# Chanuk-Yang/Deep_Continuous_Fusion_for_Multi-Sensor_3D_Object_Detection

Hardware: AMD Instinct MI355X
Metric: frames/sec (train step) 100k-pt LiDAR + 1242x375 RGB (higher is better)
Workload: dtype bf16; 1 GPU; cfg2: grid 32x704x800, 100000 pts/frame, 1242x375 RGB, ResNet-18 image stream, K=3 fusion x4 sites, eval-mode BN (reference F4), batch 2/GPU; global_batch=2, parallelism=dp1, loss_sampling=compat, conv_chain=False

## Files before the change

### deep_continuous_fusion_for_multi-sensor_3d_object_detection_amd/_hip.py

```python
import ctypes
import os
import subprocess

import numpy as np
import torch

_HERE = os.path.dirname(os.path.abspath(__file__))
LIB_PATH = os.environ.get("DCF_HIP_LIB") or os.path.join(_HERE, "libdcf_hip.so")
CSRC = os.path.join(_HERE, "csrc")

F32, BF16, F16 = 0, 1, 2
VOXEL_COMPAT, VOXEL_ACCUM, VOXEL_COMPAT_ROUNDS, VOXEL_OCCUPANCY = 0, 1, 2, 3
PROJ_COMPAT, PROJ_CORRECT = 0, 1

c_int, c_float, c_i64, c_size_t, c_void_p = ctypes.c_int, ctypes.c_float, ctypes.c_int64, ctypes.c_size_t, ctypes.c_void_p
P = c_void_p

SIGNATURES = {
    "dcf_last_error": (ctypes.c_char_p, []),
    "dcf_version": (c_int, []),
    "dcf_set_option": (c_int, [ctypes.c_char_p, ctypes.c_char_p]),
    "dcf_prof_enable": (c_int, [c_int]),
    "dcf_prof_reset": (c_int, []),
    "dcf_prof_calibrate": (c_int, [P, c_int]),
    "dcf_prof_read": (c_int, [P, P, P, P, c_int]),
    "dcf_prof_read2": (c_int, [P, P, P, P, P, c_int]),
    "dcf_compact_workspace_bytes": (c_size_t, [c_int]),
    "dcf_range_filter": (c_int, [P, c_int, P, P, P, P, P, P]),
    "dcf_voxelize_workspace_bytes": (c_size_t, [c_int, c_int, c_int]),
    "dcf_voxelize": (c_int, [P, c_int, P, P, c_int, c_int, c_int, c_int, P, P, P]),
    "dcf_voxelize_batch": (c_int, [P, P, c_int, P, P, c_int, c_int, c_int, P, P, P]),
    "dcf_voxelize_batch_nhwc": (c_int, [c_int, P, P, c_int, P, P, c_int, c_int, c_int, P, P, P]),
    "dcf_project_filter": (c_int, [P, c_int, P, P, c_float, c_float, c_int, P, P, P, P, P, P]),
    "dcf_project_filter_batch": (c_int, [P, P, c_int, P, P, c_float, c_float, c_int, P, P, c_int, P, P, P]),
    "dcf_knn_workspace_bytes": (c_size_t, [c_int, c_int, c_int]),
    "dcf_knn_bev": (c_int, [P, P, c_int, c_int, c_int, c_int, c_int, c_float, c_float, c_float, c_float, c_float, P, P, P]),
    "dcf_knn_bev_batch": (c_int, [P, P, c_int, c_int, c_int, c_int, c_int, c_int, c_float, c_float, c_float, c_float, c_float, P, P, c_size_t, P]),
    "dcf_knn_bev_sites": (c_int, [P, P, c_int, c_int, c_int, P, c_int, c_float, c_float, c_float, c_float, c_float, P]),
    "dcf_knn_bev_batch_shared": (c_int, [P, P, c_int, c_int, c_int, c_int, c_int, c_int, c_int, c_int, c_int, c_float, c_float, c_float, c_float, c_float, P, P, c_size_t, P, c_size_t, P]),
    "dcf_nchw_to_nhwc": (c_int, [c_int, P, P, c_int, c_int, c_int, c_int, P]),
    "dcf_nhwc_to_nchw": (c_int, [c_int, P, P, c_int, c_int, c_int, c_int, P]),
    "dcf_image_to_nhwc4": (c_int, [c_int, P, P, c_int, c_int, c_int, P]),
    "dcf_conv2d_fwd": (c_int, [c_int, P, P, P, P, P] + [c_int] * 12 + [P]),
    "dcf_conv2d_fwd_rowscale": (c_int, [c_int, P, P, P, P, P, P] + [c_int] * 12 + [P]),
    "dcf_conv2d_dgrad": (c_int, [c_int, P, P, P, P, P] + [c_int] * 11 + [P]),
    "dcf_conv2d_dgrad_halfres": (c_int, [c_int, P, P, P, P, P, P] + [c_int] * 11 + [P]),
    "dcf_conv3x3_chain_supported": (c_int, [c_int] * 6),
    "dcf_conv3x3_chain_workspace_bytes": (c_size_t, [c_int] * 6),
    "dcf_conv3x3_chain": (c_int, [c_int, P, c_int, c_int, c_int, c_int, c_int, c_int, P, P]),
    "dcf_fp8_act_scale": (c_int, [c_float, P]),
    "dcf_cast_fp8": (c_int, [c_int, P, P, P, P, c_i64, P]),
    "dcf_weight_prep_fp8": (c_int, [P, P, c_int, c_int, P, P, P, P, P, c_float, P]),
    "dcf_conv2d_fwd_fp8": (c_int, [c_int, P, P, P, P, P, P, P, P, P, P] + [c_int] * 12 + [P]),
    "dcf_conv2d_wgrad_splits": (c_int, [c_int] * 8),
    "dcf_conv2d_wgrad": (c_int, [c_int, P, P, P, P, c_int] + [c_int] * 11 + [P]),
    "dcf_conv2d_wgrad_groupable": (c_int, [c_int] * 10),
    "dcf_conv2d_wgrad_group": (c_int, [P, c_int, P]),
    "dcf_stem7x7_fwd": (c_int, [c_int, P, P, P, P] + [c_int] * 7 + [P]),
    "dcf_stem7x7_wgrad": (c_int, [c_int, P, P, P, P, c_int] + [c_int] * 6 + [P]),
    "dcf_weight_prep": (c_int, [c_int, P, c_int, P, P, P, P, c_float, P]),
    "dcf_wgrad_finalize": (c_int, [P, c_int, c_int, P, P, P, P, P, P, c_float, P]),
    "dcf_eval_score_filter": (c_int, [P, c_int, c_int, c_int, c_float, c_int, P, P, P]),
    "dcf_eval_nms_workspace_bytes": (c_size_t, [c_int]),
    "dcf_eval_nms": (c_int, [P, P, c_int, c_int, ctypes.c_double, P, P, P, P]),
    "dcf_eval_match": (c_int, [P, c_int, P, c_int, P, c_int, P, P]),
    "dcf_wgrad_finalize_rows": (c_int, [P, c_int, P, P, P, P, P, P, P, c_float, P]),
    "dcf_bn_workspace_bytes": (c_size_t, [c_int]),
    "dcf_bn_train_fwd": (c_int, [c_int, P, P, P, P, P, P, P, P, P, c_i64, c_int, c_float, c_float, c_int, P, P]),
    "dcf_bn_train_bwd": (c_int, [c_int, P, P, P, P, P, P, P, P, c_i64, c_int, P, P]),
    "dcf_relu_bwd_chansum": (c_int, [c_int, P, P, P, c_i64, c_int, c_int, P]),
    "dcf_resize_bilinear_fwd": (c_int, [c_int, P, P, P] + [c_int] * 7 + [P]),
    "dcf_resize_bilinear_bwd": (c_int, [c_int, P, P] + [c_int] * 7 + [P]),
    "dcf_maxpool3x3s2_fwd": (c_int, [c_int, P, P] + [c_int] * 6 + [P]),
    "dcf_maxpool3x3s2_bwd": (c_int, [c_int, P, P, P, P] + [c_int] * 6 + [P]),
    "dcf_maxpool3x3s2_fwd_idx": (c_int, [c_int, P, P, P] + [c_int] * 6 + [P]),
    "dcf_maxpool3x3s2_bwd_idx": (c_int, [c_int, P, P, P] + [c_int] * 6 + [P]),
    "dcf_head_fwd": (c_int, [c_int, P, c_int, P, P, c_int, c_int, c_int, P]),
    "dcf_head_bwd": (c_int, [c_int, P, c_int, P, P, P, P, c_int, c_int, c_int, P]),
    "dcf_point_sample_fwd": (c_int, [c_int, P, c_int, c_int, c_int, P, P, c_int, P, P]),
    "dcf_point_sample_bwd": (c_int, [c_int, P, c_int, c_int, c_int, P, P, c_int, P, P]),
    "dcf_point_sample_fwd_batch": (c_int, [c_int, P, c_int, c_int, c_int, P, c_i64, P, c_int, P, c_int, P]),
    "dcf_point_sample_bwd_batch": (c_int, [c_int, P, c_int, c_int, c_int, P, c_i64, P, c_int, P, c_int, P]),
    "dcf_fusion_gather_fwd_batch": (c_int, [c_int, P, c_i64, P, c_i64, P, c_int, c_int, c_int, c_int, c_float, c_float, c_float, c_float, P, P, c_int, P, P, c_int, P]),
    "dcf_fusion_gather_bwd_inv_batch": (c_int, [c_int, P, c_i64, P, c_i64, P, P, c_i64, P, P, c_int, c_int, c_int, c_int, c_float, c_float, c_float, c_float, P, P, c_int, P, P, P, P, P, c_int, P]),
    "dcf_fusion_gather_fwd": (c_int, [c_int, P, P, P, c_int, c_int, c_int, c_int, c_float, c_float, c_float, c_float, P, P, c_int, P, P, P]),
    "dcf_fusion_gather_bwd": (c_int, [c_int, P, P, P, c_int, c_int, c_int, c_int, c_float, c_float, c_float, c_float, P, P, c_int, P, P, P, P, P]),
    "dcf_fusion_invert_workspace_bytes": (c_size_t, [c_int, c_int]),
    "dcf_fusion_invert": (c_int, [P, c_int, c_int, c_int, P, P, P, P, P]),
    "dcf_fusion_gather_bwd_pts": (c_int, [c_int, P, P, P, c_int, P, P, c_int, c_int, c_int, c_int, c_float, c_float, c_float, c_float, P, P, c_int, P, P, P, P, P]),
    "dcf_fusion_gather_bwd_workspace_bytes": (c_size_t, [c_int]),
    "dcf_fusion_gather_bwd_direct_workspace_bytes": (c_size_t, [c_int, c_int, c_int]),
    "dcf_fusion_gather_bwd_direct_batch": (c_int, [c_int, P, c_i64, P, c_i64, P, P, c_i64, P, P, c_int, c_int, c_int, c_int, c_float, c_float, c_float, c_float, P, P, c_int, P, P, P, P, P, P, c_int, P]),
    "dcf_fusion_gather_bwd_inv": (c_int, [c_int, P, P, P, P, P, P, c_int, c_int, c_int, c_int, c_float, c_float, c_float, c_float, P, P, c_int, P, P, P, P, P, P]),
    "dcf_rowscale_bias_fwd": (c_int, [c_int, P, P, P, c_i64, c_int, P]),
    "dcf_rowscale_bias_bwd": (c_int, [c_int, P, P, P, c_i64, c_int, P]),
    "dcf_relu_mask_rowscale_bwd": (c_int, [c_int, P, P, P, P, P, c_i64, c_int, P]),
    "dcf_cast": (c_int, [c_int, P, c_int, P, c_i64, P]),
    "dcf_loss_fwd_bwd": (c_int, [P, c_i64, P, c_i64, P, P, P, c_int, c_int, c_float, c_int, P, P, c_i64, P, c_i64, P]),
    "dcf_loss_sample_rand": (ctypes.c_uint32, [ctypes.c_uint64, c_int, c_int, c_int, c_int]),
# ... 187 lines not shown
```

### deep_continuous_fusion_for_multi-sensor_3d_object_detection_amd/backend_hip.py

```python
import ctypes
import os

import numpy as np
import torch

from . import _hip as H
from . import ops

BN_EPS = 1e-5


class HipBackend(object):
    def __init__(self, plan, params, grads, buffers, dtype, fp8_min_cin=0, fp8_min_blocks=512):
        if not params.is_cuda:
            raise H.DcfError("the HIP hot path needs CUDA/HIP tensors (got %s); there is no CPU fallback" % params.device)
        H.lib()
        self.plan, self.params, self.grads, self.buffers = plan, params, grads, buffers
        self.dtype = H.dtype_code(dtype)
        self.tdtype = H.torch_dtype(self.dtype)
        self.es = 4 if self.dtype == H.F32 else 2
        self.dev = params.device
        self._fus_dws = {}
        self._wtab = {}
        self._chain_ok, self._chain_ws, self._chain_tab = {}, {}, {}
# ... 327 lines not shown
    def can_chain(self, shape, n):
        if not self.chain_enabled or n < 2 or self.bn_train or self.has_fp8 or self.dtype == H.F32:
            return False
        if os.environ.get("DCF_CHAIN") != "force":
            import torch.distributed as dist
            if dist.is_available() and dist.is_initialized() and dist.get_world_size() > 1:
                return False
        key = tuple(shape)
        ok = self._chain_ok.get(key)
        if ok is None:
            B, Hh, W, C = key
            ok = self._chain_ok[key] = ops.conv3x3_chain_supported(self.dtype, B, Hh, W, C, 1)
        return ok

    def _chain(self, x, layers, flip):
        B, Hh, W, C = x.shape
        key = (B, Hh, W, C)
        ws = self._chain_ws.get(key)
        if ws is None:
            ws = self._chain_ws[key] = ops.conv3x3_chain_workspace(self.dtype, B, Hh, W, C, H.CHAIN_MAX_LAYERS, x.device)
        outs, cur, pos = [], x, 0
        while pos < len(layers):
            part = layers[pos:pos + H.CHAIN_MAX_LAYERS]
            fix = []
            for (w, sh, r, m, relu) in part:
                r = (outs[r] if r < pos else r - pos) if type(r) is int else r
                m = (outs[m] if m < pos else m - pos) if type(m) is int else m
                fix.append((w, sh, r, m, relu))
            tab = self._chain_tab.get(len(fix))
            if tab is None:
                tab = self._chain_tab[len(fix)] = (H.ChainLayer * len(fix))()
            got = ops.conv3x3_chain(self.dtype, cur, fix, flip, ws, tab)
            outs.extend(got)
            cur = got[-1]
            pos += len(part)
        return outs

    def chain_fwd(self, x, specs):
        outs = self._chain(x, [(self._wbase + L.wfwd_off, self._shift(L), r, None, relu) for (L, r, relu) in specs], 0)
        shp = (x.shape[0], x.shape[1], x.shape[2])
        for (L, _, _) in specs:
            L.out_shape = shp
        return outs

    def chain_dgrad(self, g, specs):
        for (L, _, _) in specs:
            if L.wdgrad_off < 0:
                raise H.DcfError("layer %s was planned without an input gradient" % L.name)
        return self._chain(g, [(self._wbase + L.wdgrad_off, None, r, m, False) for (L, r, m) in specs], 1)

    def shortcut_dgrad(self, Ld, dd, L1, g1, in_shape, mask=None):
        if L1.wdgrad_off < 0 or Ld.wdgrad_off < 0:
            raise H.DcfError("layer %s was planned without an input gradient" % L1.name)
        B, Hq, Wq, _ = dd.shape
        gq = ops.conv2d_dgrad(self.dtype, dd, self._w(Ld, True), None, (B, Hq, Wq, in_shape[3]), 1, 1, 1, 0)
        return ops.conv2d_dgrad_halfres(self.dtype, g1, self._w(L1, True), None, gq, in_shape, L1.kh, L1.kw, L1.stride, L1.pad, mask)

    def _gs(self, L):
        return self._gsbase + 4 * L.gsum_off if (L.bn is not None and not self.bn_train) else None

    def _flush_wgrads(self):
        q = self._wq
        if not q:
            return
        key = tuple([t[0].idx for t in q])
        ent = self._wtab.get(key)
        shapes = [t[1].shape for t in q]
        sig = (self.bn_train, self._slbase, self._gsbase, tuple([(t[0].nsplit, t[0].slab_off, t[0].gsum_off) for t in q]))
        if ent is None or ent[1] != shapes or ent[2] != sig:
            items = (H.WgradItem * len(q))()
            for i, (L, x, gy) in enumerate(q):
                B, Hh, W, Cin = x.shape
                items[i] = H.WgradItem(self.dtype, L.nsplit, 0, 0, self._slbase + 4 * L.slab_off, self._gs(L), B, Hh, W, Cin, L.cout_pad, L.kh, L.kw, L.stride, L.pad, 0)
            if len(self._wtab) > 16:
                self._wtab.clear()
            ent = self._wtab[key] = (items, shapes, sig)
        items = ent[0]
        for i, (L, x, gy) in enumerate(q):
            it = items[i]
            it.x = x.data_ptr()
            it.gy = gy.data_ptr()
        H.call("dcf_conv2d_wgrad_group", ctypes.addressof(items), len(q), H.stream_ptr())
        self._wq = []

    _wq = []
    _fus_ws = None
    _gp_pool = None
    _group = os.environ.get("DCF_WGRAD_GROUP", "1") != "0"
    _fusion_pts = os.environ.get("DCF_FUSION_PTS", "0") == "1"
    _fusion_direct = os.environ.get("DCF_FUSION_DIRECT", "1") != "0"

    deterministic = False
    _det_ws = None

    def _det_workspace(self, key, make):
        if self._det_ws is None:
            self._det_ws = {}
        ws = self._det_ws.get(key)
        if ws is None:
            ws = self._det_ws[key] = make()
        return ws

    def conv_wgrad(self, L, x, gy, defer=True):
        if self._group and defer and L.kind != "stem":
            q = self.__dict__.get("_wq")
            if q is None:
                q = self._wq = []
            q.append((L, x, gy))
            return
# ... 181 lines not shown
```

### deep_continuous_fusion_for_multi-sensor_3d_object_detection_amd/engine.py

```python
import os

import numpy as np
import torch

FUSION_INV = os.environ.get("DCF_FUSION_INV", "1")
FUSED_SITE_MASK = os.environ.get("DCF_FUSED_SITE_MASK", "1") != "0"
HALFRES_SHORTCUT = os.environ.get("DCF_HALFRES_SHORTCUT", "1") != "0"


class ConvLayer(object):

    def __init__(self, idx, name, cin, cout, kh, kw, stride, pad, bn=None, kind="conv", need_dgrad=True, names=None):
        self.idx, self.name, self.bn, self.kind = idx, name, bn, kind
        self.cin, self.cout, self.kh, self.kw, self.stride, self.pad = cin, cout, kh, kw, stride, pad
        self.cout_pad = (cout + 31) // 32 * 32
        self.need_dgrad = need_dgrad
        self.names = names or [name]
        self.w_off = self.gamma_off = self.beta_off = self.mean_off = self.var_off = -1
        self.out_shape = None

    @property
    def taps(self):
        return self.kh * self.kw

# ... 23 lines not shown
    @staticmethod
    def physical_shape(shape, layout):
        if layout == "ohwi":
            O, I, kh, kw = shape
            return (O, kh, kw, I)
        if layout == "stem":
            return (shape[0], 7, 8, 4)
        return tuple(shape)

    @staticmethod
    def view(flat, shape, off, n, layout):
        seg = flat[off:off + n]
        if layout == "ohwi":
            O, I, kh, kw = shape
            return seg.view(O, kh, kw, I).permute(0, 3, 1, 2)
        if layout == "stem":
            return seg.view(shape[0], 7, 8, 4)[:, :, :7, :3].permute(0, 3, 1, 2)
        return seg.view(shape)


class Block(object):

    def __init__(self, conv1, conv2, down=None):
        self.conv1, self.conv2, self.down = conv1, conv2, down
        self.saved = None
        self.next_conv = None

    def forward(self, K, x, save=True):
        r = K.conv_fwd(self.down, x, None, False) if self.down is not None else x
        y1 = K.conv_fwd(self.conv1, x, None, True, self.conv2)
        y = K.conv_fwd(self.conv2, y1, r, True, self.next_conv)
        x._f8 = y1._f8 = None
        self.saved = (x, y1, y) if save else None
        return y

    def backward(self, K, g, extra=None, need_gx=True, g_masked=False, prev=None):
        x, y1, y = self.saved
        self.saved = None
        g2 = g if g_masked else K.relu_mask(g, y)
        d2 = K.bn_bwd(self.conv2, g2)
        K.conv_wgrad(self.conv2, y1, d2)
        g1 = K.bn_bwd(self.conv1, K.conv_dgrad(self.conv2, d2, tuple(y1.shape), None, y1))
        return self.backward_tail(K, x, g2, g1, extra, need_gx, prev)

    def backward_tail(self, K, x, g2, g1, extra, need_gx, prev):
        K.conv_wgrad(self.conv1, x, g1)
        pm = x if prev is not None else None
        if self.down is not None:
            dd = K.bn_bwd(self.down, g2)
            K.conv_wgrad(self.down, x, dd)
            if not need_gx:
                return None
            d, c = self.down, self.conv1
            if (extra is None and HALFRES_SHORTCUT and d.kh == 1 and d.kw == 1 and d.stride == 2 and d.pad == 0
                    and c.kh == 3 and c.stride == 2 and c.pad == 1):
                return K.shortcut_dgrad(d, dd, c, g1, tuple(x.shape), pm)
            gx = K.conv_dgrad(self.down, dd, tuple(x.shape), extra)
            return K.conv_dgrad(self.conv1, g1, tuple(x.shape), gx, pm)
        if not need_gx:
            return None
        assert extra is None, "an identity-shortcut block cannot take an extra gradient"
        return K.conv_dgrad(self.conv1, g1, tuple(x.shape), g2, pm)


def blocks_forward(K, blocks, x, save=True):
    n = len(blocks)
    ok = (n >= 1 and getattr(K, "can_chain", None) is not None and all(type(b) is Block for b in blocks)
          and all(b.down is None and b.conv1.stride == 1 for b in blocks[1:]))
    if ok:
        b0 = blocks[0]
        strided = b0.down is not None or b0.conv1.stride != 1 or b0.conv1.cin != b0.conv1.cout
        nchain = 2 * n - 1 if strided else 2 * n
        B, Hh, W, _ = x.shape
        s0 = b0.conv1.stride
        shape = (B, (Hh + 2 - 3) // s0 + 1, (W + 2 - 3) // s0 + 1, b0.conv1.cout) if strided else tuple(x.shape)
        ok = nchain >= 2 and all(L.kh == 3 and L.kw == 3 and L.pad == 1 and L.cout == L.cout_pad == shape[3]
                                 for b in blocks for L in (b.conv1, b.conv2)) and K.can_chain(shape, nchain)
    if not ok:
        for b in blocks:
            x = b.forward(K, x, save)
        return x
    specs, ins = [], []
    if strided:
        r = K.conv_fwd(b0.down, x, None, False) if b0.down is not None else x
        y1 = K.conv_fwd(b0.conv1, x, None, True)
        x0 = y1
        specs.append((b0.conv2, r, True))
        first = 1
    else:
        x0 = x
        first = 0
    xin = len(specs) - 1
    for b in blocks[first:]:
        specs.append((b.conv1, None, True))
        specs.append((b.conv2, xin if xin >= 0 else x, True))
        xin = len(specs) - 1
    outs = K.chain_fwd(x0, specs)
    if save:
        k = 0
        if strided:
            b0.saved = (x, y1, outs[0])
            k = 1
        prev = outs[0] if strided else x
        for b in blocks[first:]:
            b.saved = (prev, outs[k], outs[k + 1])
            prev = outs[k + 1]
            k += 2
    else:
        for b in blocks:
# ... 488 lines not shown
```

### deep_continuous_fusion_for_multi-sensor_3d_object_detection_amd/ops.py

```python
import ctypes

import numpy as np
import torch

from . import _hip as H


def _chk(t, name):
    if not (isinstance(t, torch.Tensor) and t.is_cuda and t.is_contiguous()):
        raise H.DcfError("%s must be a contiguous CUDA tensor" % name)
    return t


def conv_out_size(n, k, s, p):
    return (n + 2 * p - k) // s + 1


def nchw_to_nhwc(x, dtype):
    B, C, Hh, W = x.shape
    _chk(x, "x")
    y = torch.empty((B, Hh, W, C), dtype=H.torch_dtype(dtype), device=x.device)
    H.call("dcf_nchw_to_nhwc", dtype, x, y, B, C, Hh, W, H.stream_ptr())
    return y

# ... 22 lines not shown
    H.call("dcf_conv2d_fwd", dtype, x, w, shift, res, y, B, Hh, W, Cin, Ho, Wo, cout, kh, kw, stride, pad, int(relu),
           H.stream_ptr())
    return y


def conv2d_fwd_rowscale(dtype, x, w, shift, rowscale, res, relu, cout):
    B, Hh, W, Cin = x.shape
    if rowscale.numel() != B * Hh * W or rowscale.dtype != torch.float32:
        raise H.DcfError("conv2d_fwd_rowscale: rowscale must be fp32 with one entry per output pixel")
    y = torch.empty((B, Hh, W, cout), dtype=x.dtype, device=x.device)
    H.call("dcf_conv2d_fwd_rowscale", dtype, x, w, shift, _chk(rowscale, "rowscale"), res, y, B, Hh, W, Cin, Hh, W, cout, 1, 1, 1, 0, int(relu),
           H.stream_ptr())
    return y


def fp8_act_scale(amax):
    import ctypes
    out = ctypes.c_float(0.0)
    H.call("dcf_fp8_act_scale", float(amax), ctypes.addressof(out))
    return float(out.value)


def cast_fp8(dtype, x, amax_prev=None, amax_cur=None):
    x8 = torch.empty(x.shape, dtype=torch.uint8, device=x.device)
    H.call("dcf_cast_fp8", dtype, x, x8, amax_prev, amax_cur, x.numel(), H.stream_ptr())
    return x8


def conv2d_fwd_fp8(out_dtype, x8, w8, wscale, xamax, shift, res, kh, kw, stride, pad, relu, cout, want_y8=False, y8amax=None, y8cur=None):
    B, Hh, W, Cin = x8.shape
    Ho, Wo = conv_out_size(Hh, kh, stride, pad), conv_out_size(W, kw, stride, pad)
    y = torch.empty((B, Ho, Wo, cout), dtype=H.torch_dtype(out_dtype), device=x8.device)
    y8 = torch.empty((B, Ho, Wo, cout), dtype=torch.uint8, device=x8.device) if want_y8 else None
    H.call("dcf_conv2d_fwd_fp8", out_dtype, x8, w8, wscale, xamax, shift, res, y, y8, y8amax, y8cur, B, Hh, W, Cin, Ho, Wo, cout, kh, kw,
           stride, pad, int(relu), H.stream_ptr())
    return (y, y8) if want_y8 else y


def conv2d_dgrad(dtype, gy, wt, res, in_shape, kh, kw, stride, pad, mask=None):
    B, Hh, W, Cin = in_shape
    _, Ho, Wo, Cout = gy.shape
    gx = torch.empty((B, Hh, W, Cin), dtype=gy.dtype, device=gy.device)
    H.call("dcf_conv2d_dgrad", dtype, gy, wt, res, mask, gx, B, Hh, W, Cin, Ho, Wo, Cout, kh, kw, stride, pad, H.stream_ptr())
    return gx


def conv2d_dgrad_halfres(dtype, gy, wt, res, resq, in_shape, kh, kw, stride, pad, mask=None):
    B, Hh, W, Cin = in_shape
    _, Ho, Wo, Cout = gy.shape
    if tuple(resq.shape) != (B, (Hh + 1) // 2, (W + 1) // 2, Cin):
        raise H.DcfError("conv2d_dgrad_halfres: resq %s does not sit on the even sub-grid of %s" % (tuple(resq.shape), tuple(in_shape)))
    gx = torch.empty((B, Hh, W, Cin), dtype=gy.dtype, device=gy.device)
    H.call("dcf_conv2d_dgrad_halfres", dtype, gy, wt, res, resq, mask, gx, B, Hh, W, Cin, Ho, Wo, Cout, kh, kw, stride, pad, H.stream_ptr())
    return gx


def conv3x3_chain_supported(dtype, B, Hh, W, C, nlayers):
    return bool(H.lib().dcf_conv3x3_chain_supported(dtype, B, Hh, W, C, nlayers))


def conv3x3_chain_workspace(dtype, B, Hh, W, C, nlayers, device):
    n = H.lib().dcf_conv3x3_chain_workspace_bytes(dtype, B, Hh, W, C, nlayers)
    if n == 0:
        raise H.DcfError("conv3x3_chain: unsupported shape %s x %d layers" % ((B, Hh, W, C), nlayers))
    return torch.zeros((n // 4,), dtype=torch.int32, device=device)


def conv3x3_chain(dtype, x, layers, flip, ws, table=None):
    B, Hh, W, C = x.shape
    n = len(layers)
    outs = [torch.empty((B, Hh, W, C), dtype=x.dtype, device=x.device) for _ in range(n)]
    tab = table if table is not None else (H.ChainLayer * n)()
    cur = x.data_ptr()
    for l, (w, shift, res, mask, relu) in enumerate(layers):
        it = tab[l]
        it.x = cur
        it.w = H._ptr(w)
        it.shift = H._ptr(shift)
        it.res = outs[res].data_ptr() if type(res) is int else H._ptr(res)
        it.mask = outs[mask].data_ptr() if type(mask) is int else H._ptr(mask)
        cur = it.y = outs[l].data_ptr()
        it.relu = 1 if relu else 0
    import ctypes
    H.call("dcf_conv3x3_chain", dtype, ctypes.addressof(tab), n, B, Hh, W, C, int(flip), ws, H.stream_ptr())
    return outs


def conv3x3_chain_status(ws):
    return int(ws[1].item())


def conv2d_wgrad_splits(B, Ho, Wo, Cin, Cout, kh, kw, stride=1):
    return H.lib().dcf_conv2d_wgrad_splits(B, Ho, Wo, Cin, Cout, kh, kw, stride)


def conv2d_wgrad(dtype, x, gy, slabs, nsplit, kh, kw, stride, pad, gsum=None):
    B, Hh, W, Cin = x.shape
    _, Ho, Wo, Cout = gy.shape
    H.call("dcf_conv2d_wgrad", dtype, x, gy, slabs, gsum, nsplit, B, Hh, W, Cin, Ho, Wo, Cout, kh, kw, stride, pad, H.stream_ptr())
    return slabs


def stem7x7_fwd(dtype, img4, w, shift, relu, cout, Hh, W):
    B = img4.shape[0]
    Ho, Wo = conv_out_size(Hh, 7, 2, 3), conv_out_size(W, 7, 2, 3)
    y = torch.empty((B, Ho, Wo, cout), dtype=img4.dtype, device=img4.device)
# ... 562 lines not shown
```

### include/dcf_hip.h

```cpp
#ifndef DCF_HIP_H
#define DCF_HIP_H

#include <stddef.h>
#include <stdint.h>

#ifdef __cplusplus
extern "C" {
#endif

typedef void *dcf_stream_t;

enum { DCF_OK = 0, DCF_EINVAL = -1, DCF_ELAUNCH = -2, DCF_EUNSUPPORTED = -3 };
enum { DCF_F32 = 0, DCF_BF16 = 1, DCF_F16 = 2 };
enum { DCF_VOXEL_COMPAT = 0, DCF_VOXEL_ACCUM = 1, DCF_VOXEL_COMPAT_ROUNDS = 2,
       DCF_VOXEL_OCCUPANCY = 3  };
enum { DCF_PROJ_COMPAT = 0, DCF_PROJ_CORRECT = 1 };

const char *dcf_last_error(void);
int dcf_version(void);
int dcf_set_option(const char *name, const char *value);
int dcf_prof_enable(int on);
int dcf_prof_reset(void);
int dcf_prof_calibrate(dcf_stream_t stream, int n);
int dcf_prof_read(char *names , double *total_ms, int64_t *calls, double *work, int cap);
// ... 8 lines not shown
int dcf_voxelize(const float *pts, int n, const float *lim, const float *aff, int Cz, int L, int W,
                 int mode, float *grid, void *owner_ws, dcf_stream_t stream);
#define DCF_MAX_VOXEL_BATCH 8
int dcf_voxelize_batch(const float *const *pts, const int *n, int B, const float *lim, const float *aff, int Cz, int L, int W,
                       float *grids, void *owner_ws, dcf_stream_t stream);
int dcf_voxelize_batch_nhwc(int dtype, const float *const *pts, const int *n, int B, const float *lim, const float *aff, int Cz, int L,
                            int W, void *x_nhwc, void *owner_ws, dcf_stream_t stream);

int dcf_project_filter(const float *pts, int n, const float *lim, const float *crt, float ulim, float vlim,
                       int mode, float *uv_out, float *xyz_out, int32_t *src_out, int32_t *count_dev,
                       void *ws, dcf_stream_t stream);
int dcf_project_filter_batch(const float *const *pts, const int *n, int B, const float *lim, const float *crt, float ulim, float vlim,
                             int mode, float *uv_out, float *xyz_out, int rows, int32_t *count_dev, void *ws, dcf_stream_t stream);

size_t dcf_knn_workspace_bytes(int n_max, int h, int w);
int dcf_knn_bev(const float *xyz, const int32_t *count_dev, int n_max, int K, int h, int w, int stride,
                float xs, float xo, float ys, float yo, float rmax2, int32_t *idx_out, void *ws,
                dcf_stream_t stream);
int dcf_knn_bev_batch(const float *xyz, const int32_t *count_dev, int B, int n_max, int K, int h, int w, int stride,
                      float xs, float xo, float ys, float yo, float rmax2, int32_t *idx_out, void *ws, size_t ws_stride_bytes,
                      dcf_stream_t stream);

int dcf_knn_bev_batch_shared(const float *xyz, const int32_t *count_dev, int B, int n_max, int K, int h, int w, int stride,
                             int fine_h, int fine_w, int fine_stride, float xs, float xo, float ys, float yo, float rmax2,
                             int32_t *idx_out, void *ws, size_t ws_stride_bytes, const void *ws_fine, size_t ws_fine_stride_bytes,
                             dcf_stream_t stream);

typedef struct { int32_t h, w, stride, fine; int32_t *idx_out; void *ws; size_t ws_stride_bytes; } dcf_knn_site;
int dcf_knn_bev_sites(const float *xyz, const int32_t *count_dev, int B, int n_max, int K, const dcf_knn_site *sites, int nsites,
                      float xs, float xo, float ys, float yo, float rmax2, dcf_stream_t stream);

#define DCF_MAX_KNN_MAPS 32
typedef struct { const int32_t *idx; int32_t h, w; } dcf_knn_map;
size_t dcf_fusion_invert_workspace_bytes(int n_max, int nmaps);
int dcf_fusion_invert(const dcf_knn_map *maps, int nmaps, int K, int n_max, int32_t *start, int32_t *ent_pix, int32_t *ent_pt,
                      void *ws, dcf_stream_t stream);

int dcf_nchw_to_nhwc(int dtype, const float *x, void *y, int B, int C, int H, int W, dcf_stream_t stream);
int dcf_nhwc_to_nchw(int dtype, const void *x, float *y, int B, int C, int H, int W, dcf_stream_t stream);
int dcf_image_to_nhwc4(int dtype, const uint8_t *img, void *y, int B, int H, int W, dcf_stream_t stream);

int dcf_conv2d_fwd(int dtype, const void *x, const void *w, const float *shift, const void *res, void *y,
                   int B, int H, int W, int Cin, int Ho, int Wo, int Cout, int kh, int kw, int stride, int pad,
                   int relu, dcf_stream_t stream);
int dcf_conv2d_fwd_rowscale(int dtype, const void *x, const void *w, const float *shift, const float *rowscale, const void *res,
                            void *y, int B, int H, int W, int Cin, int Ho, int Wo, int Cout, int kh, int kw, int stride, int pad,
                            int relu, dcf_stream_t stream);
int dcf_conv2d_dgrad(int dtype, const void *gy, const void *wt, const void *res, const void *mask, void *gx,
                     int B, int H, int W, int Cin, int Ho, int Wo, int Cout, int kh, int kw, int stride, int pad,
                     dcf_stream_t stream);
int dcf_conv2d_dgrad_halfres(int dtype, const void *gy, const void *wt, const void *res, const void *resq,
                             const void *mask, void *gx, int B, int H, int W, int Cin, int Ho, int Wo, int Cout,
                             int kh, int kw, int stride, int pad, dcf_stream_t stream);
#define DCF_CHAIN_MAX_LAYERS 24
typedef struct {
    const void *x, *w;
    const float *shift;
    const void *res, *mask;
    void *y;
    int32_t relu, pad_;
} dcf_chain_layer;
int dcf_conv3x3_chain_supported(int dtype, int B, int H, int W, int C, int nlayers);
size_t dcf_conv3x3_chain_workspace_bytes(int dtype, int B, int H, int W, int C, int nlayers);
int dcf_conv3x3_chain(int dtype, const dcf_chain_layer *layers, int nlayers, int B, int H, int W, int C, int flip,
                      void *ws, dcf_stream_t stream);
int dcf_conv2d_wgrad_splits(int B, int Ho, int Wo, int Cin, int Cout, int kh, int kw, int stride);
int dcf_conv2d_wgrad(int dtype, const void *x, const void *gy, float *slabs, float *gsum, int nsplit,
                     int B, int H, int W, int Cin, int Ho, int Wo, int Cout, int kh, int kw, int stride, int pad,
                     dcf_stream_t stream);
typedef struct {
    int32_t dtype, nsplit;
    const void *x, *gy;
    float *slabs, *gsum;
    int32_t B, H, W, Cin, Cout, kh, kw, stride, pad, pad_;
} dcf_wgrad_item;
int dcf_conv2d_wgrad_groupable(int dtype, int B, int H, int W, int Cin, int Cout, int kh, int kw, int stride, int pad);
int dcf_conv2d_wgrad_group(const dcf_wgrad_item *items, int n, dcf_stream_t stream);
int dcf_stem7x7_fwd(int dtype, const void *img4, const void *w, const float *shift, void *y,
                    int B, int H, int W, int Ho, int Wo, int Cout, int relu, dcf_stream_t stream);
int dcf_stem7x7_wgrad(int dtype, const void *img4, const void *gy, float *slabs, float *gsum, int nsplit,
                      int B, int H, int W, int Ho, int Wo, int Cout, dcf_stream_t stream);

typedef struct dcf_conv_param {
    int64_t w_off;
    int64_t gamma_off;
    int64_t beta_off;
    int64_t mean_off;
    int64_t var_off;
    int64_t wfwd_off;
    int64_t wdgrad_off;
    int64_t shift_off;
    int64_t slab_off;
    int64_t gsum_off;
    int32_t cout, cin, taps, cout_pad;
    int32_t nsplit, flags, pad0, pad1;
} dcf_conv_param;
int dcf_weight_prep(int dtype, const dcf_conv_param *table, int nconv, const float *params, const float *buffers,
                    void *warena, float *ssarena, float eps, dcf_stream_t stream);
int dcf_wgrad_finalize(const dcf_conv_param *table, int nconv, int max_cout, const float *params, const float *buffers,
                       const float *ssarena, const float *slabs, const float *gsum, float *grads, float eps,
                       dcf_stream_t stream);
int dcf_wgrad_finalize_rows(const dcf_conv_param *table, int nconv, const int32_t *cout_host, const float *params, const float *buffers,
                            const float *ssarena, const float *slabs, const float *gsum, float *grads, float eps,
                            dcf_stream_t stream);

int dcf_fp8_act_scale(float amax, float *scale);
// ... 153 lines not shown
```

Measured before the change: 380.3 frames/s.

## Fuse stride-2 block-head dgrad of 3x3 conv and 1x1 shortcut into one kernel

Result: slower. 301.0 frames/s (-20.8%).

```diff
diff --git a/deep_continuous_fusion_for_multi-sensor_3d_object_detection_amd/_hip.py b/deep_continuous_fusion_for_multi-sensor_3d_object_detection_amd/_hip.py
--- a/deep_continuous_fusion_for_multi-sensor_3d_object_detection_amd/_hip.py
+++ b/deep_continuous_fusion_for_multi-sensor_3d_object_detection_amd/_hip.py
@@ -10,6 +10,7 @@
 CSRC = os.path.join(_HERE, "csrc")
 
 F32, BF16, F16 = 0, 1, 2
+EUNSUPPORTED = -3
 VOXEL_COMPAT, VOXEL_ACCUM, VOXEL_COMPAT_ROUNDS, VOXEL_OCCUPANCY = 0, 1, 2, 3
 PROJ_COMPAT, PROJ_CORRECT = 0, 1
 
@@ -45,6 +46,7 @@
     "dcf_conv2d_fwd_rowscale": (c_int, [c_int, P, P, P, P, P, P] + [c_int] * 12 + [P]),
     "dcf_conv2d_dgrad": (c_int, [c_int, P, P, P, P, P] + [c_int] * 11 + [P]),
     "dcf_conv2d_dgrad_halfres": (c_int, [c_int, P, P, P, P, P, P] + [c_int] * 11 + [P]),
+    "dcf_conv_s2_block_dgrad": (c_int, [c_int, P, P, P, P, P, P, P] + [c_int] * 5 + [P]),
     "dcf_conv3x3_chain_supported": (c_int, [c_int] * 6),
     "dcf_conv3x3_chain_workspace_bytes": (c_size_t, [c_int] * 6),
     "dcf_conv3x3_chain": (c_int, [c_int, P, c_int, c_int, c_int, c_int, c_int, c_int, P, P]),
diff --git a/deep_continuous_fusion_for_multi-sensor_3d_object_detection_amd/backend_hip.py b/deep_continuous_fusion_for_multi-sensor_3d_object_detection_amd/backend_hip.py
--- a/deep_continuous_fusion_for_multi-sensor_3d_object_detection_amd/backend_hip.py
+++ b/deep_continuous_fusion_for_multi-sensor_3d_object_detection_amd/backend_hip.py
@@ -403,9 +403,17 @@
     def shortcut_dgrad(self, Ld, dd, L1, g1, in_shape, mask=None):
         if L1.wdgrad_off < 0 or Ld.wdgrad_off < 0:
             raise H.DcfError("layer %s was planned without an input gradient" % L1.name)
+        gx = self.block_head_dgrad(Ld, dd, L1, g1, in_shape, None, mask)
+        if gx is not None:
+            return gx
         B, Hq, Wq, _ = dd.shape
         gq = ops.conv2d_dgrad(self.dtype, dd, self._w(Ld, True), None, (B, Hq, Wq, in_shape[3]), 1, 1, 1, 0)
         return ops.conv2d_dgrad_halfres(self.dtype, g1, self._w(L1, True), None, gq, in_shape, L1.kh, L1.kw, L1.stride, L1.pad, mask)
+
+    def block_head_dgrad(self, Ld, dd, L1, g1, in_shape, extra=None, mask=None):
+        if L1.wdgrad_off < 0 or Ld.wdgrad_off < 0:
+            raise H.DcfError("layer %s was planned without an input gradient" % L1.name)
+        return ops.conv_s2_block_dgrad(self.dtype, g1, self._w(L1, True), dd, self._w(Ld, True), extra, mask, in_shape)
 
     def _gs(self, L):
         return self._gsbase + 4 * L.gsum_off if (L.bn is not None and not self.bn_train) else None
diff --git a/deep_continuous_fusion_for_multi-sensor_3d_object_detection_amd/csrc/conv_s2d.hip b/deep_continuous_fusion_for_multi-sensor_3d_object_detection_amd/csrc/conv_s2d.hip
--- /dev/null
+++ b/deep_continuous_fusion_for_multi-sensor_3d_object_detection_amd/csrc/conv_s2d.hip
@@ -0,0 +1,309 @@
+#include <stdlib.h>
+
+#include <algorithm>
+#include <type_traits>
+
+#include "dcf_common.h"
+#include "conv_common.h"
+
+namespace {
+
+struct S2dArgs {
+    const char *g1;
+    const char *dd;
+    const char *w1;
+    const char *wd;
+    const char *extra;
+    const char *mask;
+    char *gx;
+    int B, H, W, Ho, Wo;
+    int txn, tyn;
+    int ntiles;
+    unsigned qbytes, xbytes;
+};
+
+typedef unsigned s2d_u32x4 __attribute__((ext_vector_type(4)));
+
+template <typename T> __device__ __forceinline__ float round_store(float v);
+template <> __device__ __forceinline__ float round_store<bf16_t>(float v) { return bf2f(f2bf(v)); }
+template <> __device__ __forceinline__ float round_store<f16_t>(float v) { return (float)(_Float16)v; }
+
+template <typename T, int NBUF>
+__global__ void __launch_bounds__(256) __attribute__((amdgpu_waves_per_eu(NBUF == 2 ? 3 : 2, NBUF == 2 ? 3 : 2))) k_conv_s2d(S2dArgs a)
+{
+    static_assert(DT<T>::size == 2, "16-bit element types only");
+    constexpr int TQ = 2, TW = 32;
+    constexpr int PW = 34;
+    constexpr int RB = 128;
+    constexpr int PPP = 1024 / RB;
+    constexpr int G1PX = (TQ + 1) * PW, DDPX = TQ * PW;
+    constexpr int G1P = (G1PX + PPP - 1) / PPP, DDP = (DDPX + PPP - 1) / PPP;
+    constexpr int NPIECE = G1P + DDP;
+    constexpr int PXW = (NPIECE + 3) / 4;
+    constexpr int KS = 4;
+    constexpr int NST = 4;
+    constexpr int CPP = RB / 16;
+    constexpr int OB = 64;
+    constexpr int DUMP = NBUF * NPIECE;
+    constexpr int AHEAD = (NBUF - 2) * (PXW + NST) + NST;
+    static_assert(NBUF >= 2 && AHEAD < 64, "vmcnt range");
+    static_assert((PW * RB) % 256 == 0, "row pitch");
+    static_assert((NBUF * NPIECE + 1) * 1024 * (NBUF == 2 ? 3 : 2) <= 160 * 1024, "LDS: two workgroups per CU (three with a two-slot ring)");
+    __shared__ __attribute__((aligned(1024))) char lds[(NBUF * NPIECE + 1) * 1024];
+
+    const int tid = threadIdx.x, lane = tid & 63;
+    const int wid = __builtin_amdgcn_readfirstlane(tid >> 6);
+    const int q = wid >> 1, par = wid & 1;
+    const int r = lane & 31, h = lane >> 5;
+
+    const int chunk = (a.ntiles + 7) >> 3;
+    const int wpx = gridDim.x >> 3;
+    const int chunk_lo = (blockIdx.x & 7) * chunk, chunk_hi = min(chunk_lo + chunk, a.ntiles);
+    int t = chunk_lo + (blockIdx.x >> 3);
+    if (t >= chunk_hi) return;
+
+    const __amdgpu_buffer_rsrc_t srcG = __builtin_amdgcn_make_buffer_rsrc((void *)a.g1, 0, a.qbytes, 0x00020000);
+    const __amdgpu_buffer_rsrc_t srcD = __builtin_amdgcn_make_buffer_rsrc((void *)a.dd, 0, a.qbytes, 0x00020000);
+    const __amdgpu_buffer_rsrc_t srcE = __builtin_amdgcn_make_buffer_rsrc((void *)(a.extra ? a.extra : a.gx), 0, a.xbytes, 0x00020000);
+    const __amdgpu_buffer_rsrc_t srcM = __builtin_amdgcn_make_buffer_rsrc((void *)(a.mask ? a.mask : a.gx), 0, a.xbytes, 0x00020000);
+    const __amdgpu_buffer_rsrc_t dstY = __builtin_amdgcn_make_buffer_rsrc((void *)a.gx, 0, a.xbytes, 0x00020000);
+    constexpr unsigned OOB = 0xFFFFFF00u;
+    const unsigned lds0 = lds_addr(lds);
+
+    uint4 wreg[6 * KS];
+    {
+        const int tapE[6] = {4, 3, 5, 0, 0, 0}, tapO[6] = {1, 7, 0, 2, 6, 8};
+        const char *w1p = a.w1 + (size_t)r * (9 * RB) + h * 16;
+        const char *wdp = a.wd + (size_t)r * RB + h * 16;
+#pragma unroll
+        for (int s = 0; s < 6; ++s) {
+            const char *p = par ? w1p + tapO[s] * RB : (s == 3 ? wdp : w1p + tapE[s] * RB);
+#pragma unroll
+            for (int ks = 0; ks < KS; ++ks) wreg[s * KS + ks] = *reinterpret_cast<const uint4 *>(p + ks * 32);
+        }
+    }
+
+    __builtin_amdgcn_s_waitcnt(0x0F70);
+
+    auto colkey = [](int cc) { return (cc >> 1) & 7; };
+    int relo[PXW];
+#pragma unroll
+    for (int j = 0; j < PXW; ++j) {
+        const int p = wid + 4 * j;
+        const bool isd = p >= G1P;
+        const int i = (isd ? p - G1P : p) * PPP + lane / CPP;
+        const int rr_ = i / PW, cc_ = i - rr_ * PW;
+        const bool ok = p < NPIECE && (isd ? (i < DDPX && cc_ < TW) : (i < G1PX && cc_ < TW + 1));
+        relo[j] = ok ? (rr_ * a.Wo + cc_) * RB + (((lane % CPP) ^ colkey(cc_)) << 4) : -1;
+    }
+    auto issue_tile = [&](int tile, int buf) __attribute__((always_inline)) {
+        const int tx = tile % a.txn, tq = tile / a.txn;
+        const int ty = tq % a.tyn, b = tq / a.tyn;
+        const int i0 = ty * TQ, j0 = tx * TW;
+        const bool inner = tile < chunk_hi && i0 + TQ + 1 <= a.Ho && j0 + TW + 1 <= a.Wo;
+        const int org = ((b * a.Ho + i0) * a.Wo + j0) * RB;
+        if (inner) {
+#pragma unroll
+            for (int j = 0; j < PXW; ++j) {
+                const int p = wid + 4 * j;
+                glds16(p >= G1P ? srcD : srcG, relo[j] >= 0 ? (unsigned)(org + relo[j]) : OOB,
+                       __builtin_amdgcn_readfirstlane(lds0 + (p < NPIECE ? buf * NPIECE + p : DUMP) * 1024));
+            }
+        } else {
+            const int ln = opaque(lane);
+#pragma unroll
+            for (int j = 0; j < PXW; ++j) {
+                const int p = wid + 4 * j;
+                const int i = (p >= G1P ? p - G1P : p) * PPP + ln / CPP;
+                const int rr_ = i / PW, cc_ = i - rr_ * PW;
+                const bool live = tile < chunk_hi && relo[j] >= 0 && i0 + rr_ < a.Ho && j0 + cc_ < a.Wo;
+                glds16(p >= G1P ? srcD : srcG, live ? (unsigned)(org + relo[j]) : OOB,
+                       __builtin_amdgcn_readfirstlane(lds0 + (p < NPIECE ? buf * NPIECE + p : DUMP) * 1024));
+            }
+        }
+    };
+
+    int xoff[2][KS];
+#pragma unroll
+    for (int dj = 0; dj < 2; ++dj)
+#pragma unroll
+        for (int ks = 0; ks < KS; ++ks) xoff[dj][ks] = (r + dj) * RB + (((2 * ks + h) ^ colkey(r + dj)) << 4);
+
+    const bool has_extra = a.extra != nullptr, has_mask = a.mask != nullptr;
+
+#pragma unroll
+    for (int d = 0; d < NBUF - 1; ++d) {
+        issue_tile(t + d * wpx, d);
+#pragma unroll
+        for (int k = 0; k < NST; ++k) {
+            const s2d_u32x4 z = {0u, 0u, 0u, 0u};
+            asm volatile("buffer_store_dwordx4 %0, %1, %2, 0 offen\n\ts_nop 1" ::"v"(z), "v"(OOB), "s"(dstY) : "memory");
+        }
+    }
+    int buf = 0;
+    for (;;) {
+        const int tx = t % a.txn, tq = t / a.txn;
+        const int ty = tq % a.tyn, b = tq / a.tyn;
+        const int tn = t + wpx;
+        const int oh = 2 * (ty * TQ + q) + par, ow = 2 * (tx * TW + r);
+        const int mpix = (b * a.H + oh) * a.W + ow;
+        const unsigned offA = (oh < a.H && ow < a.W) ? (unsigned)mpix * OB + 16 * h : OOB;
+        const unsigned offB = (oh < a.H && ow + 1 < a.W) ? (unsigned)(mpix + 1) * OB + 16 * h : OOB;
+        asm volatile("s_waitcnt lgkmcnt(0)" ::: "memory");
+        wait_vmcnt<AHEAD>();
+        __builtin_amdgcn_s_barrier();
+        uint4 ev[4], mv[4];
+        if (has_extra) {
+#pragma unroll
+            for (int k = 0; k < 4; ++k)
+                ev[k] = __builtin_bit_cast(uint4, __builtin_amdgcn_raw_buffer_load_b128(srcE, (k & 2 ? offB : offA) + 32 * (k & 1), 0, 0));
+        }
+        if (has_mask) {
+#pragma unroll
+            for (int k = 0; k < 4; ++k)
+                mv[k] = __builtin_bit_cast(uint4, __builtin_amdgcn_raw_buffer_load_b128(srcM, (k & 2 ? offB : offA) + 32 * (k & 1), 0, 0));
+        }
+        issue_tile(t + (NBUF - 1) * wpx, buf == 0 ? NBUF - 1 : buf - 1);
+        const char *tg = lds + buf * (NPIECE * 1024) + q * PW * RB;
+        const char *td = tg + G1P * 1024;
+        f32x16 acc[3];
+#pragma unroll
+        for (int j = 0; j < 3; ++j)
+#pragma unroll
+            for (int k = 0; k < 16; ++k) acc[j][k] = 0.f;
+        auto tap = [&](f32x16 &c, int s, const char *p, int dj) __attribute__((always_inline)) {
+            uint4 fb[KS];
+#pragma unroll
+            for (int ks = 0; ks < KS; ++ks) fb[ks] = *reinterpret_cast<const uint4 *>(p + xoff[dj][ks]);
+#pragma unroll
+            for (int ks = 0; ks < KS; ++ks) Mma<T>::run(wreg[s * KS + ks], fb[ks], c);
+        };
+        if (par == 0) {
+            tap(acc[0], 0, tg, 0);
+            tap(acc[1], 1, tg, 1);
+            tap(acc[2], 3, td, 0);
+            asm volatile("" ::: "memory");
+            tap(acc[1], 2, tg, 0);
+        } else {
+            tap(acc[0], 0, tg + PW * RB, 0);
+            tap(acc[1], 2, tg + PW * RB, 1);
+            asm volatile("" ::: "memory");
+            tap(acc[0], 1, tg, 0);
+            tap(acc[1], 3, tg + PW * RB, 0);
+            asm volatile("" ::: "memory");
+            tap(acc[1], 4, tg, 1);
+            asm volatile("" ::: "memory");
+            tap(acc[1], 5, tg, 0);
+        }
+        acc_rows8(acc[0]);
+        acc_rows8(acc[1]);
+        if (par == 0) {
+            acc_rows8(acc[2]);
+            if (!has_extra) {
+#pragma unroll
+                for (int k = 0; k < 16; ++k) acc[0][k] += round_store<T>(acc[2][k]);
+            }
+        } else {
+#pragma unroll
+            for (int k = 0; k < 16; ++k) acc[2][k] = 0.f;
+        }
+        if (has_extra) {
+#pragma unroll
+            for (int c = 0; c < 2; ++c)
+#pragma unroll
+                for (int p = 0; p < 2; ++p) {
+                    const uint4 e4 = ev[2 * c + p];
+                    const unsigned ew[4] = {e4.x, e4.y, e4.z, e4.w};
+#pragma unroll
+                    for (int e = 0; e < 4; ++e) {
+                        float lo, hi;
+                        unpack2<T>(ew[e], lo, hi);
+                        const float blo = c == 0 ? acc[2][8 * p + 2 * e] : 0.f, bhi = c == 0 ? acc[2][8 * p + 2 * e + 1] : 0.f;
+                        acc[c][8 * p + 2 * e] += round_store<T>(blo + lo);
+                        acc[c][8 * p + 2 * e + 1] += round_store<T>(bhi + hi);
+                    }
+                }
+        }
+        if (has_mask) {
+#pragma unroll
+            for (int c = 0; c < 2; ++c)
+#pragma unroll
+                for (int p = 0; p < 2; ++p) {
+                    const uint4 m4 = mv[2 * c + p];
+                    const unsigned mw[4] = {m4.x, m4.y, m4.z, m4.w};
+#pragma unroll
+                    for (int e = 0; e < 4; ++e) {
+                        float lo, hi;
+                        unpack2<T>(mw[e], lo, hi);
+                        if (!(lo > 0.f)) acc[c][8 * p + 2 * e] = 0.f;
+                        if (!(hi > 0.f)) acc[c][8 * p + 2 * e + 1] = 0.f;
+                    }
+                }
+        }
+#pragma unroll
+        for (int c = 0; c < 2; ++c)
+#pragma unroll
+            for (int p = 0; p < 2; ++p) {
+                float v[8];
+#pragma unroll
+                for (int k = 0; k < 8; ++k) v[k] = acc[c][8 * p + k];
+                uint4 pk;
+                if constexpr (std::is_same<T, bf16_t>::value) {
+                    pk = make_uint4(pack2bf(v[0], v[1]), pack2bf(v[2], v[3]), pack2bf(v[4], v[5]), pack2bf(v[6], v[7]));
+                } else {
+                    typedef _Float16 h16x8 __attribute__((ext_vector_type(8)));
+                    h16x8 hv;
+#pragma unroll
+                    for (int k = 0; k < 8; ++k) hv[k] = (_Float16)v[k];
+                    pk = __builtin_bit_cast(uint4, hv);
+                }
+                const s2d_u32x4 d = {pk.x, pk.y, pk.z, pk.w};
+                __builtin_amdgcn_raw_buffer_store_b128(d, dstY, (int)((c ? offB : offA) + 32 * p), 0, 0);
+            }
+        if (tn >= chunk_hi) break;
+        t = tn;
+        buf = buf + 1 == NBUF ? 0 : buf + 1;
+    }
+}
+
+}
+
+extern "C" int dcf_conv_s2_block_dgrad(int dtype, const void *g1, const void *w1t, const void *dd, const void *wdt, const void *extra,
+                                       const void *mask, void *gx, int B, int H, int W, int Cin, int Cout, dcf_stream_t stream)
+{
+    DCF_REQUIRE(dtype == DCF_F32 || dtype == DCF_BF16 || dtype == DCF_F16, "dcf_conv_s2_block_dgrad: unsupported dtype %d", dtype);
+    DCF_REQUIRE(g1 && w1t && dd && wdt && gx, "dcf_conv_s2_block_dgrad: null pointer");
+    DCF_REQUIRE(B > 0 && H > 0 && W > 0, "dcf_conv_s2_block_dgrad: empty tensor (B=%d H=%d W=%d)", B, H, W);
+    DCF_REQUIRE(Cin > 0 && Cin % 32 == 0, "dcf_conv_s2_block_dgrad: Cin must be a multiple of 32 (Cin=%d)", Cin);
+    DCF_REQUIRE(Cout > 0 && Cout % 32 == 0, "dcf_conv_s2_block_dgrad: Cout must be a multiple of 32 (Cout=%d)", Cout);
+    const int Ho = (H + 1) / 2, Wo = (W + 1) / 2;
+    const int es = dtype == DCF_F32 ? 4 : 2;
+    DCF_REQUIRE((int64_t)B * H * W * Cin * es < 0xFFFFFF00ll && (int64_t)B * Ho * Wo * Cout * es < 0xFFFFFF00ll,
+                "dcf_conv_s2_block_dgrad: tensor exceeds the 4 GiB buffer-descriptor range");
+    static DcfOpt on_o("S2DGRAD"), minpix_o("S2DGRAD_MIN_PIX");
+    const char *on = on_o.str(), *mp = minpix_o.str();
+    if (on && atoi(on) == 0) return DCF_EUNSUPPORTED;
+    if (dtype == DCF_F32 || Cin != 32 || Cout != 64) return DCF_EUNSUPPORTED;
+    const int64_t npix = (int64_t)B * H * W;
+    if (npix < (mp ? atoll(mp) : 200000ll)) return DCF_EUNSUPPORTED;
+    if (npix * Cin * 2 >= (1ll << 31) || (int64_t)B * Ho * Wo * Cout * 2 >= (1ll << 31)) return DCF_EUNSUPPORTED;
+    S2dArgs a;
+    a.g1 = (const char *)g1; a.dd = (const char *)dd; a.w1 = (const char *)w1t; a.wd = (const char *)wdt;
+    a.extra = (const char *)extra; a.mask = (const char *)mask; a.gx = (char *)gx;
+    a.B = B; a.H = H; a.W = W; a.Ho = Ho; a.Wo = Wo;
+    a.txn = (Wo + 31) / 32; a.tyn = (Ho + 1) / 2;
+    a.ntiles = B * a.txn * a.tyn;
+    a.qbytes = (unsigned)((int64_t)B * Ho * Wo * Cout * 2);
+    a.xbytes = (unsigned)(npix * Cin * 2);
+    const int64_t nwg = std::min<int64_t>(((int64_t)a.ntiles + 7) / 8 * 8, 256 * 2);
+    const dim3 grid((unsigned)nwg);
+    const double flops = 2.0 * B * Ho * Wo * (double)Cout * Cin * (9 + 1);
+    const double bytes = 2.0 * (double)a.qbytes + (double)a.xbytes * (1 + (extra ? 1 : 0) + (mask ? 1 : 0)) + 10.0 * Cin * Cout * 2.0;
+    hipStream_t s = S(stream);
+    char name[64];
+    snprintf(name, sizeof(name), "conv_dgrad_%s<s2d,3>", dtype == DCF_F16 ? "f16" : "bf16");
+#define DCF_S2D(T_) DCF_LAUNCH_WB(name, flops, bytes, s, hipLaunchKernelGGL((k_conv_s2d<T_, 3>), grid, dim3(256), 0, s, a))
+    if (dtype == DCF_F16) DCF_S2D(f16_t); else DCF_S2D(bf16_t);
+#undef DCF_S2D
+    return DCF_OK;
+}
diff --git a/deep_continuous_fusion_for_multi-sensor_3d_object_detection_amd/engine.py b/deep_continuous_fusion_for_multi-sensor_3d_object_detection_amd/engine.py
--- a/deep_continuous_fusion_for_multi-sensor_3d_object_detection_amd/engine.py
+++ b/deep_continuous_fusion_for_multi-sensor_3d_object_detection_amd/engine.py
@@ -99,9 +99,14 @@
             if not need_gx:
                 return None
             d, c = self.down, self.conv1
-            if (extra is None and HALFRES_SHORTCUT and d.kh == 1 and d.kw == 1 and d.stride == 2 and d.pad == 0
-                    and c.kh == 3 and c.stride == 2 and c.pad == 1):
+            head = (d.kh == 1 and d.kw == 1 and d.stride == 2 and d.pad == 0 and c.kh == 3 and c.kw == 3 and c.stride == 2 and c.pad == 1)
+            if extra is None and HALFRES_SHORTCUT and head:
                 return K.shortcut_dgrad(d, dd, c, g1, tuple(x.shape), pm)
+            fused = getattr(K, "block_head_dgrad", None) if (head and extra is not None) else None
+            if fused is not None:
+                gx = fused(d, dd, c, g1, tuple(x.shape), extra, pm)
+                if gx is not None:
+                    return gx
             gx = K.conv_dgrad(self.down, dd, tuple(x.shape), extra)
             return K.conv_dgrad(self.conv1, g1, tuple(x.shape), gx, pm)
         if not need_gx:
diff --git a/deep_continuous_fusion_for_multi-sensor_3d_object_detection_amd/ops.py b/deep_continuous_fusion_for_multi-sensor_3d_object_detection_amd/ops.py
--- a/deep_continuous_fusion_for_multi-sensor_3d_object_detection_amd/ops.py
+++ b/deep_continuous_fusion_for_multi-sensor_3d_object_detection_amd/ops.py
@@ -98,6 +98,25 @@
         raise H.DcfError("conv2d_dgrad_halfres: resq %s does not sit on the even sub-grid of %s" % (tuple(resq.shape), tuple(in_shape)))
     gx = torch.empty((B, Hh, W, Cin), dtype=gy.dtype, device=gy.device)
     H.call("dcf_conv2d_dgrad_halfres", dtype, gy, wt, res, resq, mask, gx, B, Hh, W, Cin, Ho, Wo, Cout, kh, kw, stride, pad, H.stream_ptr())
+    return gx
+
+
+def conv_s2_block_dgrad(dtype, g1, w1t, dd, wdt, extra, mask, in_shape):
+    B, Hh, W, Cin = in_shape
+    Cout = g1.shape[3]
+    q = (B, (Hh + 1) // 2, (W + 1) // 2, Cout)
+    if tuple(g1.shape) != q or tuple(dd.shape) != q:
+        raise H.DcfError("conv_s2_block_dgrad: g1 %s / dd %s are not the half-resolution grid %s of %s" % (tuple(g1.shape), tuple(dd.shape), q, tuple(in_shape)))
+    for t, name in ((extra, "extra"), (mask, "mask")):
+        if t is not None and tuple(t.shape) != tuple(in_shape):
+            raise H.DcfError("conv_s2_block_dgrad: %s %s does not have the input's shape %s" % (name, tuple(t.shape), tuple(in_shape)))
+    gx = torch.empty((B, Hh, W, Cin), dtype=g1.dtype, device=g1.device)
+    rc = H.fn("dcf_conv_s2_block_dgrad")(dtype, H._ptr(g1), H._ptr(w1t), H._ptr(dd), H._ptr(wdt), H._ptr(extra), H._ptr(mask), H._ptr(gx),
+                                         B, Hh, W, Cin, Cout, H.stream_ptr())
+    if rc == H.EUNSUPPORTED:
+        return None
+    if rc != 0:
+        H.fail("dcf_conv_s2_block_dgrad", rc)
     return gx
 
 
diff --git a/include/dcf_hip.h b/include/dcf_hip.h
--- a/include/dcf_hip.h
+++ b/include/dcf_hip.h
@@ -84,6 +84,8 @@
 int dcf_conv2d_dgrad_halfres(int dtype, const void *gy, const void *wt, const void *res, const void *resq,
                              const void *mask, void *gx, int B, int H, int W, int Cin, int Ho, int Wo, int Cout,
                              int kh, int kw, int stride, int pad, dcf_stream_t stream);
+int dcf_conv_s2_block_dgrad(int dtype, const void *g1, const void *w1t, const void *dd, const void *wdt, const void *extra,
+                            const void *mask, void *gx, int B, int H, int W, int Cin, int Cout, dcf_stream_t stream);
 #define DCF_CHAIN_MAX_LAYERS 24
 typedef struct {
     const void *x, *w;
```
